# Meryx/ComputeRayTracer

Measured on AMD Instinct MI355X. Metric: Mrays/sec (+ HBM GB/s vs peak), 1080p 250k-tri scene, 1/2/4/8 MI355X, higher is better.
Workload: dtype f32; 1 GPU; S2 atrium250k: 253952 triangles + cornell walls/light, 1920x1080, 64 spp per step (BASELINE config 3)

## Files before the change

### computeraytracer_amd/csrc/crt_api.cpp

```cpp
#include <hip/hip_runtime.h>

#include <algorithm>
#include <cfloat>
#include <cmath>
#include <cstdarg>
#include <cstdio>
#include <cstdlib>
#include <cstring>
#include <chrono>
#include <string>
#include <thread>
#include <vector>

#include "../../include/crt.h"
#include "crt_bvh.h"
#include "crt_device.h"
#include "crt_math.h"

namespace crt {
hipError_t launch_trace(const TraceParams &P, bool count, bool brute, hipStream_t stream);
hipError_t launch_trace_adaptive(const TraceParams &P, const AsTiles &A, bool count, bool brute, hipStream_t stream);
hipError_t wf_launch_resolve_adaptive(const WfParams &P, const AsTiles &A, uint32_t call_end, hipStream_t s);
hipError_t as_launch_select(const AsParams &A, bool compact, hipStream_t s);
hipError_t as_launch_commit(uint32_t *counts, const uint32_t *active, uint32_t n_active, uint32_t samples, hipStream_t s);
// ... 101 lines not shown
    Bvh4 bvh4;
    Bvh4Q bvh4q;
    Bvh8Q bvh8q;
    int quantize = 1;
    int wf_width = 4;

    DevBuf<unsigned char> d_raw;
    DevBuf<float4> d_prim, d_primD, d_nodes, d_nodes4, d_lights;
    DevBuf<int> w_overflow;
    DevBuf<uint4> d_nodes4q, d_nodes8q;
    DevBuf<uint32_t> d_slot_of_index;
    DevBuf<float> d_spectra, d_cie;
    DevScene sc{};

    uint32_t x0 = 0, y0 = 0, tw = 0, th = 0;
    uint32_t band = 0x40000000u, stride = 1, phase = 0;
    DevBuf<float4> d_accum;
    DevBuf<uchar4> d_rgba;
    DevBuf<uchar4> d_frames;
    uint32_t frame_ring = 0;
    std::vector<uint8_t> frame_batch;
    hipStream_t read_stream = nullptr;
    uint32_t ring_from = 1;
    uint32_t resolved_upto = 0;
    float4 *accum_bound = nullptr;
    uchar4 *rgba_bound = nullptr;
    uint32_t sample = 0;
    uint32_t published = 0;
    uint32_t pending = 0;
    bool in_publish = false;
    int wf_cohort = 16;

    DevBuf<unsigned long long> d_counters;
    bool counting = false;
    float last_ms = 0.0f;
    uint32_t last_launches = 0;
    bool last_timed = false;
    uint32_t spp_per_launch = 0;

    int pipeline = 1;
    uint32_t wf_pool = 0;
    uint32_t wf_waves_per_cu = 0;
    int num_cu = 0;
    DevBuf<float4> w_ray_o, w_ray_d, w_sh_d, w_beta, w_radiance, w_nee, w_staging[kWfRing], w_recA, w_recB;
    DevBuf<uint4> w_rng, w_misc, w_recC;
    DevBuf<float2> w_hit;
    DevBuf<uint32_t> w_vis, w_dead, w_tea;
    static constexpr int kMaxPipes = 4;
    int wf_pipes = 2;
    int wf_defer = 1;
    int wf_tail_walk = 1;
    int wf_gen_blocks = 128;
    int wf_trace_form = 2;
    int wf_chunk = 1;
    int wf_ahead = 3;
    int wf_ring = 32;
    int wf_pool_spp = 8;
    double wf_feed = 1.0;
    WfRun *run = nullptr;
    uint32_t wf_finish_at = 32768;
    uint32_t wf_flush_at = 4096;
    uint32_t wf_side_ppw = 64, wf_flush_ppw = 4;
    DevBuf<WfCtl> w_ctl[kMaxPipes];
    DevBuf<WfWorkQ> w_wq;
    static constexpr int kStatusSlots = 64;
    WfStatus *h_status[kMaxPipes] = {};
    WfStatus *d_status[kMaxPipes] = {};
    hipEvent_t ev_status[kMaxPipes][kStatusSlots] = {};
    hipEvent_t ev_done[kMaxPipes][kStatusSlots] = {};
    uint32_t *h_dropped = nullptr;
    bool wf_host_ready = false;
    hipStream_t pipe_stream[kMaxPipes] = {};
    hipStream_t pub_stream = nullptr;
    static constexpr int kFinishStreams = 3;
    hipStream_t fin_stream[kFinishStreams] = {};
    hipEvent_t ev_fin[kFinishStreams] = {};
    int fin_next = 0;
    hipEvent_t ev_fork = nullptr, ev_join[kMaxPipes] = {}, ev_pub_join[kMaxPipes] = {};
    hipEvent_t ev_evict[kMaxPipes][kWfRing] = {};
    hipEvent_t ev_resolved[kWfRing] = {};
    hipEvent_t ev_pub[kWfRing] = {};
    bool time_kernels = false;
    std::vector<hipEvent_t> kev;
    float last_trace_kernel_ms = 0.0f;
    uint32_t last_trace_kernel_launches = 0;
    uint32_t last_iterations = 0;
    unsigned long long probes[8] = {0};

    DevBuf<float4> dn_gbuf;
    DevBuf<uint32_t> dn_key;
    bool dn_valid = false;
    DevBuf<float4> dn_c[2];
    DevBuf<uchar4> dn_rgba;

    float s_prims = 0.0f;
    float tree_pad = 0.0f;
    bool accel_stale = false;
    bool rf_ready = false;
    DevBuf<int> rf_lv2, rf_lv4;
    std::vector<uint32_t> rf_off2, rf_off4;
    DevBuf<uint32_t> rf_nch4, rf_cnt;
    DevBuf<float> rf_fb;

    bool as_on = false;
    bool as_broken = false;
    DevBuf<uint32_t> as_counts;
// ... 1078 lines not shown
        r.K = g.K; r.P = g.P; r.Pp = g.Pp; r.list_cap = g.list_cap;
        r.trace_blocks = (uint32_t)c->num_cu * wf_waves(c);
        r.open.clear();
        WfBatch nb;
        nb.n = n; nb.last_sample = last_sample; nb.id = 0; nb.as_commit = as ? as->commit : 0u;
        r.open.push_back(nb);
        r.seg_total[0] = work_total; r.seg_wps[0] = work_per_shard;
        for (uint32_t b = 0; b < kWfRing; b++) {
            r.queue_left[b] = false; r.consumed[b] = 0; r.resolved_recorded[b] = false;
            for (int p = 0; p < crt_ctx::kMaxPipes; p++) r.listed_until[b][p] = 0;
        }
        r.queue_left[0] = r.work_left = true;
        r.consumed_total = 0; r.rate_consumed = 0; r.rate_its = 0;
        r.per_it = (double)g.Pp;
        r.all_evicting = false; r.poll_next = 0;
        r.as = as ? AsTiles{c->as_active.p, c->as_counts.p, c->as_q.p, as->n_active} : AsTiles{};
        for (int p = 0; p < r.K; p++) {
            const uint32_t it0 = r.pipes[p].it + 2u * (uint32_t)kStatusRing;
            r.pipes[p] = WfPipe();
            r.pipes[p].it = r.pipes[p].it_first = r.pipes[p].it_confirmed = r.pipes[p].it_done = it0;
            r.pipes[p].chunk = (uint32_t)c->wf_chunk;
            WfParams &W = r.pipes[p].W;
            W.sc = c->sc;
            W.ray_o = c->w_ray_o.p; W.ray_d = c->w_ray_d.p; W.sh_d = c->w_sh_d.p; W.beta = c->w_beta.p;
            W.radiance = c->w_radiance.p; W.nee = c->w_nee.p; W.rng = c->w_rng.p; W.misc = c->w_misc.p;
            W.hit = c->w_hit.p; W.vis = c->w_vis.p;
            W.dead = c->w_dead.p + (g.list_per_pipe / 8) * (size_t)p;
            W.rearm = 0;
            W.gen_blocks = std::max(1u, std::min((uint32_t)c->wf_gen_blocks, g.list_cap / 64u));
            W.recA = c->w_recA.p + g.list_per_pipe * (size_t)p; W.recB = c->w_recB.p + g.list_per_pipe * (size_t)p;
            W.recC = c->w_recC.p + g.list_per_pipe * (size_t)p;
            for (uint32_t b = 0; b < kWfRing; b++) {
                W.staging[b] = c->w_staging[b < r.ring ? b : 0].p;
                W.side_base[b] = (b * (uint32_t)crt_ctx::kMaxPipes + (uint32_t)p) * kWfSideCap;
                W.seg[b] = WfSeg{0, 64, 0};
                W.seg_order[b] = 0;
            }
            W.batch_id = 0; W.count_alive = 0; W.keep_pool = 0; W.evict_mask = 0; W.status_out = nullptr;
            W.ctl = c->w_ctl[p].p; W.wq = c->w_wq.p;
            W.slot_base = side_slots + g.Pp * (uint32_t)p; W.reset_wq = (p == 0) ? 1u : 0u;
            W.P = g.Pp; W.x0 = c->x0; W.y0 = c->y0; W.tw = c->tw; W.th = c->th;
            W.band = c->band; W.stride = c->stride; W.phase = c->phase;
            W.tiles_x = g.tiles_x; W.tiles_y = g.tiles_y; W.npix_padded = g.npix_padded;
            W.list_cap = g.list_cap;
            W.seg[0] = WfSeg{work_total, work_per_shard, first_sample};
            W.seg_n = 1;
            W.n_samples = n;
            W.accum = accum_ptr(c); W.rgba = rgba_ptr(c);
            W.tea = c->w_tea.p;
            W.count = c->counting ? 1u : 0u;
            W.overflow_lanes = (uint32_t)c->num_cu * wf_waves(c) * 64u;
            W.stack_overflow = c->w_overflow.p + (size_t)p * W.overflow_lanes * kWfOverflowLevels;
            W.trace_form = (uint32_t)c->wf_trace_form;
            if (!c->pipe_stream[p]) {
                int least = 0, greatest = 0;
                HIPCHK(c, hipDeviceGetStreamPriorityRange(&least, &greatest));
                HIPCHK(c, hipStreamCreateWithPriority(&c->pipe_stream[p], hipStreamNonBlocking, greatest));
            }
            r.pipes[p].stream = c->pipe_stream[p];
            r.pipes[p].blocks_now = r.trace_blocks;
        }
        for (int p = 0; p < r.K; p++) r.rate_its += r.pipes[p].it_confirmed;
        HIPCHK(c, wf_launch_init(r.pipes[0].W, c->stream));
        HIPCHK(c, wf_launch_tea(r.pipes[0].W, c->w_tea.p, c->stream));
        HIPCHK(c, hipEventRecord(c->ev_fork, c->stream));
        for (int p = 0; p < r.K; p++) {
            HIPCHK(c, hipStreamWaitEvent(r.pipes[p].stream, c->ev_fork, 0));
            if (p > 0) HIPCHK(c, wf_launch_init(r.pipes[p].W, r.pipes[p].stream));
        }
        HIPCHK(c, hipStreamWaitEvent(c->pub_stream, c->ev_fork, 0));
        r.live = true;
    } else {
        rc = wf_pump(c, true);
        if (rc) return rc;
        WfBatch nb;
        nb.n = n; nb.last_sample = last_sample; nb.id = (r.open.back().id + 1u) % r.ring; nb.as_commit = as ? as->commit : 0u;
        const uint32_t id = nb.id;
        r.seg_total[id] = work_total; r.seg_wps[id] = work_per_shard;
        r.queue_left[id] = r.work_left = true;
        r.consumed[id] = 0;
        for (int p = 0; p < r.K; p++) {
            WfPipe &pp = r.pipes[p];
            nb.from_it[p] = 0xFFFFFFFFu;
            pp.W.seg[id] = WfSeg{work_total, work_per_shard, first_sample};
            pp.W.n_samples = n;
            pp.W.batch_id = id; pp.W.keep_pool = 1;
            pp.tail_bound = 0; pp.blocks_now = r.trace_blocks;
            pp.any = false; pp.chunk = (uint32_t)c->wf_chunk; pp.done = false;
            pp.dry[id] = false; pp.alive_valid[id] = false; pp.alive[id] = 0;
        }
        for (int p = 0; p < r.K; p++)
            if (r.listed_until[id][p] > r.pipes[p].it_confirmed) {
                HIPCHK(c, hipEventRecord(c->ev_pub_join[p], r.pipes[p].stream));
                HIPCHK(c, hipStreamWaitEvent(c->pub_stream, c->ev_pub_join[p], 0));
            }
        if (r.resolved_recorded[id]) HIPCHK(c, hipStreamWaitEvent(c->pub_stream, c->ev_resolved[id], 0));
        for (int p = 0; p < r.K; p++) HIPCHK(c, wf_launch_init(r.pipes[p].W, c->pub_stream));
        HIPCHK(c, hipEventRecord(c->ev_pub[id], c->pub_stream));
        nb.ready = false;
        r.open.push_back(nb);
    }
    if (!as) c->published += n;
    rc = wf_pump(c, false);
    if (rc == CRT_OK && !defer) rc = wf_flush(c);
    if (rc != CRT_OK && r.live) {
        for (int p = 0; p < crt_ctx::kMaxPipes; p++) if (c->pipe_stream[p]) (void)hipStreamSynchronize(c->pipe_stream[p]);
// ... 679 lines not shown
        c->last_trace_kernel_launches = 0;
    } else {
        HIPCHK(c, hipEventElapsedTime(&total, c->ev0, c->ev1));
        n = c->last_launches;
    }
    if (ms) *ms = total;
    if (launches) *launches = n;
    return CRT_OK;
}

int crt_accel_stats(crt_ctx *c, uint64_t out[8])
{
    if (!c || !out) return CRT_EINVAL;
    const bool wide = c->pipeline == 1 && c->accel_mode == CRT_ACCEL_BVH2 && c->bvh4.n_inner > 0;
    const bool wide8 = wide && c->bvh8q.ok;
    out[4] = wide ? (c->bvh4q.ok ? 16 : 32) : 32;
    out[5] = wide8 ? 8 : wide ? 4 : 2;
    out[6] = wide8 ? c->bvh8q.n_inner : wide ? c->bvh4.n_inner : c->bvh.n_inner;
    out[7] = (uint64_t)c->accel_builder;
    out[0] = c->bvh.n_inner; out[1] = c->bvh.n_leaves; out[2] = c->bvh.max_depth;
    out[3] = (uint64_t)c->bvh.n_inner * 64u + (uint64_t)c->bvh4.n_inner * 128u + (uint64_t)c->prims.size() * 48u;
    return CRT_OK;
}

int crt_set_option(crt_ctx *c, const char *name, int64_t value)
{
    if (!c || !name) return CRT_EINVAL;
    { int rc_ = wf_flush(c); if (rc_) return rc_; }
    if (!std::strcmp(name, "debug_fail_alloc")) { g_fail_alloc_in = value; return CRT_OK; }
    if (!std::strcmp(name, "wf_defer")) { c->wf_defer = value != 0; return CRT_OK; }
    if (!std::strcmp(name, "spp_per_launch")) { c->spp_per_launch = (uint32_t)std::max<int64_t>(0, value); return CRT_OK; }
    if (!std::strcmp(name, "pipeline")) { c->pipeline = value ? 1 : 0; return CRT_OK; }
    if (!std::strcmp(name, "quantize")) { c->quantize = value ? 1 : 0; return CRT_OK; }
    if (!std::strcmp(name, "wf_width")) { c->wf_width = value == 4 ? 4 : 8; return CRT_OK; }
    if (!std::strcmp(name, "wf_finish_at")) { c->wf_finish_at = (uint32_t)std::max<int64_t>(0, value); return CRT_OK; }
    if (!std::strcmp(name, "wf_flush_at")) { c->wf_flush_at = (uint32_t)std::max<int64_t>(0, value); return CRT_OK; }
    if (!std::strcmp(name, "wf_side_ppw")) { c->wf_side_ppw = (uint32_t)std::min<int64_t>(64, std::max<int64_t>(1, value)); return CRT_OK; }
    if (!std::strcmp(name, "wf_flush_ppw")) { c->wf_flush_ppw = (uint32_t)std::min<int64_t>(64, std::max<int64_t>(1, value)); return CRT_OK; }
    if (!std::strcmp(name, "wf_ring")) { c->wf_ring = (int)std::min<int64_t>((int64_t)kWfRing, std::max<int64_t>(2, value)); return CRT_OK; }
    if (!std::strcmp(name, "wf_chunk")) { c->wf_chunk = (int)std::min<int64_t>(16, std::max<int64_t>(1, value)); return CRT_OK; }
    if (!std::strcmp(name, "wf_cohort")) { c->wf_cohort = (int)std::min<int64_t>(256, std::max<int64_t>(1, value)); return CRT_OK; }
    if (!std::strcmp(name, "wf_ahead")) { c->wf_ahead = (int)std::min<int64_t>(32, std::max<int64_t>(2, value)); return CRT_OK; }
    if (!std::strcmp(name, "wf_pool_spp")) { c->wf_pool_spp = (int)std::min<int64_t>(64, std::max<int64_t>(1, value)); return CRT_OK; }
    if (!std::strcmp(name, "wf_feed_pct")) { c->wf_feed = (double)std::min<int64_t>(400, std::max<int64_t>(10, value)) / 100.0; return CRT_OK; }
    if (!std::strcmp(name, "wf_tail_walk")) { c->wf_tail_walk = value != 0; return CRT_OK; }
    if (!std::strcmp(name, "frame_ring")) {
        c->frame_ring = (uint32_t)std::min<int64_t>(256, std::max<int64_t>(0, value));
        c->ring_from = c->sample + 1u;
        if (c->have_scene) { HIPCHK(c, hipSetDevice(c->device)); HIPCHK(c, hipStreamSynchronize(c->stream)); return alloc_frames(c); }
        return CRT_OK;
    }
    if (!std::strcmp(name, "wf_gen_blocks")) { c->wf_gen_blocks = (int)std::min<int64_t>(4096, std::max<int64_t>(1, value)); return CRT_OK; }
    if (!std::strcmp(name, "wf_trace_form")) { c->wf_trace_form = value == 1 ? 1 : 2; return CRT_OK; }
    if (!std::strcmp(name, "wf_pipes")) { c->wf_pipes = (int)std::min<int64_t>(crt_ctx::kMaxPipes, std::max<int64_t>(1, value)); return CRT_OK; }
    if (!std::strcmp(name, "wf_pool")) { c->wf_pool = (uint32_t)std::max<int64_t>(0, value); return CRT_OK; }
    if (!std::strcmp(name, "wf_waves_per_cu")) { c->wf_waves_per_cu = (uint32_t)std::min<int64_t>(32, std::max<int64_t>(0, value)); return CRT_OK; }
    if (!std::strcmp(name, "time_kernels")) {
        c->time_kernels = value != 0; c->last_trace_kernel_launches = 0;
        HIPCHK(c, hipSetDevice(c->device));
        while (value > 1 && c->kev.size() < 2 * (size_t)std::min<int64_t>(value, 1 << 20)) {
            hipEvent_t e;
            HIPCHK(c, hipEventCreate(&e));
            c->kev.push_back(e);
        }
        return CRT_OK;
    }
    return fail(c, CRT_EINVAL, "crt_set_option: unknown option '%s'", name);
}

static int dn_check_state(crt_ctx *c, const char *what)
{
    if (!c->have_scene || c->accel_mode < 0) return fail(c, CRT_ESTATE, "%s: scene + accel required", what);
    if (c->accel_stale) return fail(c, CRT_ESTATE, "%s: primitives were updated: call crt_refit_accel or crt_build_accel first", what);
    if (c->sample == 0) return fail(c, CRT_ESTATE, "%s: no sample traced yet", what);
    if (c->band != 0x40000000u)
        return fail(c, CRT_ESTATE, "%s: not under a row-band partition (neighbouring local rows are not neighbouring image rows)", what);
    if ((size_t)c->tw * c->th != 0 && !accum_ptr(c))
        return fail(c, CRT_ENOMEM, "%s: the tile's buffers are not allocated (an earlier crt_set_tile failed)", what);
    return CRT_OK;
}

static int dn_ensure_gbuffer(crt_ctx *c)
{
    if (c->dn_valid) return CRT_OK;
    const size_t n = (size_t)c->tw * c->th;
    if (c->dn_gbuf.n < 2 * n) HIPCHK(c, c->dn_gbuf.alloc(2 * n));
    if (c->dn_key.n < n) HIPCHK(c, c->dn_key.alloc(n));
    HIPCHK(c, dn_launch_gbuffer(c->sc, c->x0, c->y0, c->tw, c->th, c->dn_gbuf.p, c->dn_key.p, c->accel_mode == CRT_ACCEL_NONE, c->stream));
    c->dn_valid = true;
    return CRT_OK;
}

int crt_denoise(crt_ctx *c, const crt_denoise_params *params, float *rgb_out, uint8_t *rgba8_out)
{
    if (!c) return CRT_EINVAL;
    const crt_denoise_params dp = params ? *params : crt_denoise_params{5u, 1.0f, 0.5f, 0.3f};
    if (dp.iterations > 10u) return fail(c, CRT_EINVAL, "crt_denoise: iterations %u > 10", dp.iterations);
    const float sig[3] = {dp.sigma_color, dp.sigma_normal, dp.sigma_plane};
    for (float v : sig)
        if (!(v > 0.0f && v <= 3.40282347e38f)) return fail(c, CRT_EINVAL, "crt_denoise: every sigma must be positive and finite");
    if (c->as_on) return as_refuse(c, "crt_denoise");
    { int rc = dn_check_state(c, "crt_denoise"); if (rc) return rc; }
    HIPCHK(c, hipSetDevice(c->device));
    { int rc_ = wf_flush(c); if (rc_) return rc_; }
    const size_t n = (size_t)c->tw * c->th;
    if (n) {
// ... 253 lines not shown
```

### computeraytracer_amd/csrc/crt_device.h

```cpp
#pragma once
#include <hip/hip_runtime.h>
#include <stdint.h>

namespace crt {

constexpr uint32_t kNoHit = 0xFFFFFFFFu;
constexpr int kStackDepth = 64;
constexpr uint32_t kNLambda = 301;
constexpr uint32_t kNCie = 471;
constexpr int CRT_NCOUNTERS_DEV = 16;

struct DevScene {
    const float4 *prim;
    const float4 *primD;
    const uint32_t *slot_of_index;
    const float4 *nodes;
    const float4 *nodes4;
    const uint4 *nodes4q;
    const uint4 *nodes8q;
    const float *spectra;
    const float *cie;
    const float4 *lights;
    uint32_t nprim;
    uint32_t npatch;
// ... 85 lines not shown
    unsigned long long rays;
    unsigned long long consumed[kWfRing];
    uint32_t left[kWfRing];
    uint32_t alive[kWfRing];
};

constexpr uint32_t kWfFinishSegs = 32;
struct WfFinishSegs {
    struct WfCtl *ctl[kWfFinishSegs];
    uint32_t base[kWfFinishSegs], batch[kWfFinishSegs];
    uint32_t n, blocks_per_seg;
};

struct WfParams {
    DevScene sc;
    float4 *ray_o, *ray_d, *sh_d, *beta, *radiance, *nee;
    uint4 *rng, *misc;
    float2 *hit;
    uint32_t *vis;
    float4 *recA, *recB;
    uint4 *recC;
    uint32_t *dead;
    uint32_t rearm;
    uint32_t gen_blocks;
    float4 *staging[kWfRing];
    uint32_t batch_id;
    WfStatus *status_out;
    uint32_t count_alive;
    uint32_t keep_pool;
    uint32_t side_base[kWfRing];
    uint32_t evict_mask;
    WfCtl *ctl;
    WfWorkQ *wq;
    WfSeg seg[kWfRing];
    uint32_t seg_order[kWfRing];
    uint32_t seg_n;
    uint32_t slot_base;
    uint32_t reset_wq;
    uint32_t P;
    uint32_t x0, y0, tw, th;
    uint32_t band, stride, phase;
    uint32_t tiles_x, tiles_y;
    uint32_t npix_padded;
    uint32_t list_cap;
    uint32_t tail_bound;
    uint32_t n_samples;
    float4 *accum;
    uchar4 *rgba;
    uchar4 *frames;
    uint32_t frame_ring;
    const uint32_t *tea;
    uint32_t count;
    uint32_t trace_form;
    int *stack_overflow;
    uint32_t overflow_lanes;
};

}
```

### computeraytracer_amd/csrc/crt_wavefront.hip

```cpp
#include "crt_shade.h"
#include <algorithm>

namespace crt {

#ifndef CRT_WF_STACK
#define CRT_WF_STACK 32
#endif
#ifndef CRT_WF_REFILL
#define CRT_WF_REFILL 24
#endif
#ifndef CRT_WF_INNER_RUN
#define CRT_WF_INNER_RUN 6
#endif
#ifndef CRT_WF_BURSTS
#define CRT_WF_BURSTS 4
#endif
#ifndef CRT_WF_BVH4
#define CRT_WF_BVH4 1
#endif
#ifndef CRT_WF_LEAF_AT
#define CRT_WF_LEAF_AT 32
#endif
#ifndef CRT_WF_SPEC
#define CRT_WF_SPEC 1
// ... 1051 lines not shown
#endif
                }
            }
        }
    }
    if (COUNT) {
        wave_add(ctl->counters[blockIdx.x % kWfShards] + CRT_CNT_NODES, c_nodes);
        wave_add(ctl->counters[blockIdx.x % kWfShards] + CRT_CNT_PRIMS, c_prims);
        if (lane == 0) {
            atomicAdd(ctl->counters[blockIdx.x % kWfShards] + 8, (unsigned long long)d_inner_it); atomicAdd(ctl->counters[blockIdx.x % kWfShards] + 9, (unsigned long long)d_inner_act);
            atomicAdd(ctl->counters[blockIdx.x % kWfShards] + 10, (unsigned long long)d_leaf_it); atomicAdd(ctl->counters[blockIdx.x % kWfShards] + 11, (unsigned long long)d_leaf_act);
            atomicAdd(ctl->counters[blockIdx.x % kWfShards] + 12, (unsigned long long)d_prim_it); atomicAdd(ctl->counters[blockIdx.x % kWfShards] + 13, (unsigned long long)d_scans); atomicAdd(ctl->counters[blockIdx.x % kWfShards] + 14, (unsigned long long)d_refill);
            atomicAdd(ctl->counters[blockIdx.x % kWfShards] + 15, (unsigned long long)d_refill_lanes);
        }
    }
}

#ifndef CRT_WF_PICK_AT
#define CRT_WF_PICK_AT 8
#endif
#ifndef CRT_WF_PKFMA
#define CRT_WF_PKFMA 0
#endif
#ifndef CRT_WF_LEAF2_AT
#define CRT_WF_LEAF2_AT 28
#endif
#ifndef CRT_WF_STALL_AT
#define CRT_WF_STALL_AT 16
#endif
constexpr int kStk2 = 16;
#ifndef CRT_WF_RING
#define CRT_WF_RING 32
#endif
constexpr uint32_t kRing2 = CRT_WF_RING;

__device__ __forceinline__ int stack_pop2(const int *stk, const int *ovf, size_t ovl, int sp)
{
    int v = stk[(sp < kStk2 ? sp : kStk2 - 1) * 64];
    if (sp >= kStk2) v = *(const volatile int *)(ovf + (size_t)(sp - kStk2) * ovl);
    return v;
}
__device__ __forceinline__ uint32_t mbcnt64(unsigned long long m)
{
    return __builtin_amdgcn_mbcnt_hi((uint32_t)(m >> 32), __builtin_amdgcn_mbcnt_lo((uint32_t)m, 0u));
}
__device__ __forceinline__ unsigned long long hit_key(float t, uint32_t index)
{
    return ((unsigned long long)f_bits(t) << 32) | (unsigned long long)(index == kNoHit ? 0xFFFFFFFFu : 0xFFFFFFFEu - index);
}

#ifndef CRT_WF_T2_WAVES
#define CRT_WF_T2_WAVES 5
#endif
template <bool COUNT>
__global__ __launch_bounds__(64, CRT_WF_T2_WAVES) void k_wf_trace2(const WfParams P, uint32_t it)
{
    __shared__ int lds_stack[kStk2 * 64];
    __shared__ float4 ring[4][kRing2];
    __shared__ uint2 ring_l[kRing2];
    __shared__ unsigned long long cell[64];
    __shared__ uint32_t cslot[64];
    __shared__ uint2 tasks[64];
    WfCtl *ctl = P.ctl;
    const uint4 *__restrict__ nodesq = P.sc.nodes4q;
    const f3 qscale = f3{P.sc.qscale[0], P.sc.qscale[1], P.sc.qscale[2]}, qbase = f3{P.sc.qbase[0], P.sc.qbase[1], P.sc.qbase[2]};
    const float4 *__restrict__ prim = P.sc.prim;
    const float4 *__restrict__ primD = P.sc.primD;
    uint32_t *__restrict__ g_vis = P.vis;
    float2 *__restrict__ g_hit = P.hit;
    const size_t cls_stride = (size_t)P.list_cap * kWfShards;
    const float4 *__restrict__ recA = P.recA + (size_t)((it & 1u) * 4u) * cls_stride;
    const float4 *__restrict__ recB = P.recB + (size_t)((it & 1u) * 4u) * cls_stride;
    const uint4 *__restrict__ recC = P.recC + (size_t)((it & 1u) * 4u) * cls_stride;
    const float hit_pad = P.sc.hit_pad;
    const int root = P.sc.root4;
    int *__restrict__ ovf = P.stack_overflow + ((size_t)blockIdx.x * 64 + lane_id());
    const size_t ovl = P.overflow_lanes;
    const uint32_t nprim = P.sc.nprim;
    const bool fetchD = ((unsigned long long)P.sc.npatch << CRT_WF_PATCH_RECOMPUTE) > (unsigned long long)nprim;
    DevScene S = P.sc;
    S.prim = prim; S.primD = primD;

    const uint32_t ringi = it & 3u;
    const uint32_t lane = lane_id();
    int *stk = lds_stack + lane;
    const float t_min = 0.001f;

    uint32_t cur_shard = blockIdx.x % kWfShards, sh_e0 = 0, sh_e1 = 0, sh_e2 = 0, sh_total = 0;
    uint32_t chunk_pos = 0, chunk_end = 0, ring_head = 0, ring_n = 0;
    bool have_shard = false, exhausted = false;
    {
        const WfShard &so = ctl->shard[ringi][cur_shard];
        sh_e0 = so.n[0]; sh_e1 = sh_e0 + so.n[1]; sh_e2 = sh_e1 + so.n[2]; sh_total = sh_e2 + so.n[3];
        have_shard = sh_total > 0u;
    }
    bool active = false;
    int pend = 0;
    f3 o = f3{0, 0, 0}, d = f3{0, 0, 0}, id = f3{0, 0, 0}, oid = f3{0, 0, 0};
    uint32_t excl = 0, slot = 0, b_index = kNoHit, b_slot = kNoHit, b_slot_in = kNoHit;
    float t_max = 0.0f;
    bool shadow = false;
    int node = kNoNode, sp = 0;
    bool gx = false, gy = false, gz = false;
    uint32_t c_nodes = 0, c_prims = 0;
    uint32_t d_inner_it = 0, d_inner_act = 0, d_leaf_it = 0, d_leaf_act = 0, d_prim_it = 0, d_refill = 0, d_refill_lanes = 0, d_scans = 0;

    for (;;) {
        const unsigned long long idle = __ballot(!active);
        const int nidle = __popcll(idle);
        if (nidle >= CRT_WF_PICK_AT) {
            if (ring_n == 0u && !exhausted) {
                for (int guard = 0; chunk_pos == chunk_end && !exhausted && guard < 2 * (int)kWfShards; guard++) {
                    if (have_shard) {
                        uint32_t base = 0;
                        if (lane == 0) base = atomicAdd(&ctl->shard[ringi][cur_shard].cur, (uint32_t)kTraceChunk);
                        base = __shfl(base, 0, 64);
                        if (base < sh_total) { chunk_pos = base; chunk_end = min(base + (uint32_t)kTraceChunk, sh_total); break; }
                        have_shard = false;
                    }
                    if (COUNT) d_scans++;
                    const WfShard &sl = ctl->shard[ringi][lane % kWfShards];
                    const uint32_t e0 = sl.n[0], e1 = e0 + sl.n[1], e2 = e1 + sl.n[2], tot = e2 + sl.n[3];
                    const uint32_t cur_l = __hip_atomic_load(&sl.cur, __ATOMIC_RELAXED, __HIP_MEMORY_SCOPE_AGENT);
                    const unsigned long long avail = __ballot(cur_l < tot);
                    if (!avail) { exhausted = true; break; }
                    const uint32_t rot = cur_shard & 63u;
                    const unsigned long long rmask = rot ? ((avail >> rot) | (avail << (64u - rot))) : avail;
                    cur_shard = ((uint32_t)(__ffsll((long long)rmask) - 1) + rot) & 63u;
                    sh_e0 = __shfl(e0, (int)cur_shard, 64); sh_e1 = __shfl(e1, (int)cur_shard, 64);
                    sh_e2 = __shfl(e2, (int)cur_shard, 64); sh_total = __shfl(tot, (int)cur_shard, 64);
                    have_shard = true;
                }
                if (chunk_pos < chunk_end) {
                    const uint32_t n = min(kRing2, chunk_end - chunk_pos);
                    bool ok = false;
                    float4 R0 = float4{0, 0, 0, 0}, R1 = R0, R2 = R0, R3 = R0;
                    uint2 RL = uint2{kNoHit, kNoHit};
                    if (lane < n) {
                        const uint32_t idx = chunk_pos + lane;
                        const size_t region = (size_t)cur_shard * P.list_cap;
                        const bool sh = idx >= sh_e1;
                        const size_t g = idx < sh_e0 ? region + idx : idx < sh_e1 ? cls_stride + region + (idx - sh_e0)
                                       : idx < sh_e2 ? 2u * cls_stride + region + (idx - sh_e1) : 3u * cls_stride + region + (idx - sh_e2);
                        const float4 ro = ldnt(&recA[g]), rd = ldnt(&recB[g]);
                        uint4 rc = uint4{0, 0, 0, 0};
                        if (sh) rc = ldnt(&recC[g]);
                        uint32_t r_slot;
                        float r_tmax;
                        ok = true;
                        if (sh) {
                            r_slot = rc.x & kWfListSlot; r_tmax = rd.w;
                            RL = uint2{rc.y, rc.z};
                        } else {
                            r_slot = f_bits(rd.w) & kWfListSlot; r_tmax = CRT_INFINITY;
                            if (f_bits(rd.w) & kWfListAlsoExt) ok = false;
                            else if (nprim == 0u) { g_hit[r_slot] = float2{r_tmax, bits_f(kNoHit)}; ok = false; }
                        }
// ... 88 lines not shown
                    else if (sp > 0) { sp--; node = stack_pop2(stk, ovf, ovl, sp); }
                    else node = kNoNode;
                }
                const f3 to = f3{__shfl(o.x, owner, 64), __shfl(o.y, owner, 64), __shfl(o.z, owner, 64)};
                const f3 td = f3{__shfl(d.x, owner, 64), __shfl(d.y, owner, 64), __shfl(d.z, owner, 64)};
                const uint32_t t_excl = (uint32_t)__shfl((int)excl, owner, 64);
                bool acc = false;
                unsigned long long key = 0;
                if (lane < T) {
                    const unsigned long long cur = cell[owner];
                    float tm = bits_f((uint32_t)(cur >> 32));
                    const uint32_t low = (uint32_t)cur;
                    uint32_t bi = low == 0xFFFFFFFFu ? kNoHit : 0xFFFFFFFEu - low;
                    const uint32_t bs0 = low == 0xFFFFFFFFu ? kNoHit : 0xFFFFFFFEu;
                    uint32_t bs = bs0;
                    if ((f_bits(A.w) & 3u) == 2u) tri_test(A, B, C, ps, to, td, t_excl, t_min, hit_pad, tm, bi, bs);
                    else {
                        if (!fetchD && (f_bits(A.w) & 3u) == 0u) { const f3 nn = normalize(cross(xyz(B), xyz(C))); D = float4{nn.x, nn.y, nn.z, dot(xyz(B), xyz(B))}; }
                        hit_test_rec<false>(A, B, C, D, hit_pad, ps, to, td, t_excl, t_min, tm, bi, bs);
                    }
                    if (COUNT && __ballot((f_bits(A.w) & 3u) != 2u) != 0ull) d_scans += 64u;
                    acc = bs != bs0;
                    if (acc) {
                        key = hit_key(tm, bi);
                        atomicMin(&cell[owner], key);
                    }
                    if (COUNT) c_prims++;
                }
                __builtin_amdgcn_fence(__ATOMIC_ACQ_REL, "wavefront");
                __builtin_amdgcn_wave_barrier();
                if (acc && cell[owner] == key) cslot[owner] = ps;
                __builtin_amdgcn_fence(__ATOMIC_ACQ_REL, "wavefront");
                __builtin_amdgcn_wave_barrier();
                if (incl) {
                    const unsigned long long v = cell[lane];
                    const uint32_t low = (uint32_t)v;
                    t_max = bits_f((uint32_t)(v >> 32));
                    b_index = low == 0xFFFFFFFFu ? kNoHit : 0xFFFFFFFEu - low;
                    b_slot = cslot[lane];
                    bool done = false;
                    if (shadow && b_slot != b_slot_in) done = true;
                    else if (node == kNoNode && pend == 0) done = true;
                    if (done) {
                        if (shadow) stnt(&g_vis[slot], (b_slot == b_slot_in) ? 1u : 0u);
                        else stnt(&g_hit[slot], float2{t_max, bits_f(b_slot)});
                        active = false;
                    }
                }
            } else {
                if (COUNT) { d_inner_it++; d_inner_act += (uint32_t)ni; }
                if (inner) {
                    float k0, k1, k2, k3;
                    int r0, r1, r2, r3;
                    const uint4 *nq = (const uint4 *)((const char *)nodesq + ((uint32_t)node << 6));
                    const uint4 Q0 = nq[0], Q1 = nq[1], Q2 = nq[2], Q3 = nq[3];
                    const uint32_t nxa = gx ? Q1.z : Q0.x, nxb = gx ? Q1.w : Q0.y, fxa = gx ? Q0.x : Q1.z, fxb = gx ? Q0.y : Q1.w;
                    const uint32_t nya = gy ? Q2.x : Q0.z, nyb = gy ? Q2.y : Q0.w, fya = gy ? Q0.z : Q2.x, fyb = gy ? Q0.w : Q2.y;
                    const uint32_t nza = gz ? Q2.z : Q1.x, nzb = gz ? Q2.w : Q1.y, fza = gz ? Q1.x : Q2.z, fzb = gz ? Q1.y : Q2.w;
#if CRT_WF_PKFMA
                    {
                        const v2f ix = v2f{id.x, id.x}, iy = v2f{id.y, id.y}, iz = v2f{id.z, id.z};
                        const v2f ox = v2f{oid.x, oid.x}, oy = v2f{oid.y, oid.y}, oz = v2f{oid.z, oid.z};
#define CRT_PK(Q, I, O) __builtin_elementwise_fma(v2f{(float)((Q) & 0xFFFFu), (float)((Q) >> 16)}, I, O)
                        const v2f tnx_a = CRT_PK(nxa, ix, ox), tnx_b = CRT_PK(nxb, ix, ox), tfx_a = CRT_PK(fxa, ix, ox), tfx_b = CRT_PK(fxb, ix, ox);
                        const v2f tny_a = CRT_PK(nya, iy, oy), tny_b = CRT_PK(nyb, iy, oy), tfy_a = CRT_PK(fya, iy, oy), tfy_b = CRT_PK(fyb, iy, oy);
                        const v2f tnz_a = CRT_PK(nza, iz, oz), tnz_b = CRT_PK(nzb, iz, oz), tfz_a = CRT_PK(fza, iz, oz), tfz_b = CRT_PK(fzb, iz, oz);
#undef CRT_PK
#define CRT_QK(K, NX, NY, NZ, FX, FY, FZ) { \
                            const float tn_ = __builtin_fmaxf(__builtin_fmaxf(NX, NY), __builtin_fmaxf(NZ, t_min)); \
                            const float tf_ = __builtin_fminf(__builtin_fminf(FX, FY), __builtin_fminf(FZ, t_max)); \
                            K = (tn_ <= tf_ * 1.0000005f) ? tn_ : 3.0e38f; }
                        CRT_QK(k0, tnx_a.x, tny_a.x, tnz_a.x, tfx_a.x, tfy_a.x, tfz_a.x)
                        CRT_QK(k1, tnx_a.y, tny_a.y, tnz_a.y, tfx_a.y, tfy_a.y, tfz_a.y)
                        CRT_QK(k2, tnx_b.x, tny_b.x, tnz_b.x, tfx_b.x, tfy_b.x, tfz_b.x)
                        CRT_QK(k3, tnx_b.y, tny_b.y, tnz_b.y, tfx_b.y, tfy_b.y, tfz_b.y)
#undef CRT_QK
                    }
#else
#define CRT_QBOX(K, NXQ, NYQ, NZQ, FXQ, FYQ, FZQ) { \
                        const float tn_ = __builtin_fmaxf(__builtin_fmaxf(fma_((float)(NXQ), id.x, oid.x), fma_((float)(NYQ), id.y, oid.y)), \
                                                          __builtin_fmaxf(fma_((float)(NZQ), id.z, oid.z), t_min)); \
                        const float tf_ = __builtin_fminf(__builtin_fminf(fma_((float)(FXQ), id.x, oid.x), fma_((float)(FYQ), id.y, oid.y)), \
                                                          __builtin_fminf(fma_((float)(FZQ), id.z, oid.z), t_max)); \
                        K = (tn_ <= tf_ * 1.0000005f) ? tn_ : 3.0e38f; }
                    CRT_QBOX(k0, nxa & 0xFFFFu, nya & 0xFFFFu, nza & 0xFFFFu, fxa & 0xFFFFu, fya & 0xFFFFu, fza & 0xFFFFu)
                    CRT_QBOX(k1, nxa >> 16, nya >> 16, nza >> 16, fxa >> 16, fya >> 16, fza >> 16)
                    CRT_QBOX(k2, nxb & 0xFFFFu, nyb & 0xFFFFu, nzb & 0xFFFFu, fxb & 0xFFFFu, fyb & 0xFFFFu, fzb & 0xFFFFu)
                    CRT_QBOX(k3, nxb >> 16, nyb >> 16, nzb >> 16, fxb >> 16, fyb >> 16, fzb >> 16)
#undef CRT_QBOX
#endif
                    r0 = (int)Q3.x; r1 = (int)Q3.y; r2 = (int)Q3.z; r3 = (int)Q3.w;
                    if (COUNT) c_nodes += 4;
#define CRT_CAS(ka, ra, kb, rb) { const bool sw_ = kb < ka; const float tk_ = sw_ ? kb : ka; kb = sw_ ? ka : kb; ka = tk_; \
                                  const int tr_ = sw_ ? rb : ra; rb = sw_ ? ra : rb; ra = tr_; }
                    CRT_CAS(k0, r0, k1, r1) CRT_CAS(k2, r2, k3, r3) CRT_CAS(k0, r0, k2, r2) CRT_CAS(k1, r1, k3, r3) CRT_CAS(k1, r1, k2, r2)
#undef CRT_CAS
                    if (k0 < 3.0e38f) {
                        if (k3 < 3.0e38f) { if (sp < kStk2) stk[sp * 64] = r3; else ovf[(size_t)(sp - kStk2) * ovl] = r3; sp++; }
                        if (k2 < 3.0e38f) { if (sp < kStk2) stk[sp * 64] = r2; else ovf[(size_t)(sp - kStk2) * ovl] = r2; sp++; }
                        if (k1 < 3.0e38f) { if (sp < kStk2) stk[sp * 64] = r1; else ovf[(size_t)(sp - kStk2) * ovl] = r1; sp++; }
                        node = r0;
                    } else if (sp > 0) {
                        sp--; node = stack_pop2(stk, ovf, ovl, sp);
                    } else {
                        node = kNoNode;
                        if (pend == 0) {
                            if (shadow) stnt(&g_vis[slot], (b_slot == b_slot_in) ? 1u : 0u);
                            else stnt(&g_hit[slot], float2{t_max, bits_f(b_slot)});
                            active = false;
                        }
                    }
                }
            }
        }
    }
    if (COUNT) {
        wave_add(ctl->counters[blockIdx.x % kWfShards] + CRT_CNT_NODES, c_nodes);
        wave_add(ctl->counters[blockIdx.x % kWfShards] + CRT_CNT_PRIMS, c_prims);
        if (lane == 0) {
            atomicAdd(ctl->counters[blockIdx.x % kWfShards] + 8, (unsigned long long)d_inner_it); atomicAdd(ctl->counters[blockIdx.x % kWfShards] + 9, (unsigned long long)d_inner_act);
            atomicAdd(ctl->counters[blockIdx.x % kWfShards] + 10, (unsigned long long)d_leaf_it); atomicAdd(ctl->counters[blockIdx.x % kWfShards] + 11, (unsigned long long)d_leaf_act);
            atomicAdd(ctl->counters[blockIdx.x % kWfShards] + 12, (unsigned long long)d_prim_it); atomicAdd(ctl->counters[blockIdx.x % kWfShards] + 13, (unsigned long long)d_scans); atomicAdd(ctl->counters[blockIdx.x % kWfShards] + 14, (unsigned long long)d_refill);
            atomicAdd(ctl->counters[blockIdx.x % kWfShards] + 15, (unsigned long long)d_refill_lanes);
        }
    }
}

template <bool COUNT>
__global__ __launch_bounds__(64) void k_wf_finish(const WfParams P, const WfFinishSegs G)
{
    __shared__ int lds_stack[kStackDepth * 64];
    const DevScene &S = P.sc;
    const uint32_t seg = blockIdx.x / G.blocks_per_seg, blk = blockIdx.x % G.blocks_per_seg;
    WfCtl *ctl = G.ctl[seg];
    int *stk = lds_stack + lane_id();
    const uint32_t j = blk * P.tail_bound + threadIdx.x;
    const uint32_t count = min(ctl->side_count[G.batch[seg]], kWfSideCap);
    if (blk == 0 && threadIdx.x == 0 && count > G.blocks_per_seg * P.tail_bound) atomicAdd(&ctl->dropped, count - G.blocks_per_seg * P.tail_bound);
    const bool mine = threadIdx.x < P.tail_bound && j < count;
    const uint32_t slot = G.base[seg] + (mine ? j : 0u);
    uint32_t flags = 0;
    if (mine) flags = P.misc[slot].y;
    bool alive = mine && (flags & kWfAlive);
    bool pend_sh = false, pend_ext = false;
    const bool wide = S.nodes4q != nullptr && S.nodes8q == nullptr;
    ShadeCnt cn;
    uint32_t c_nodes = 0, c_prims = 0;
    for (int guard = 0; guard < 512 && __ballot(alive) != 0ull; guard++) {
        if (alive) {
            const float4 ro = P.ray_o[slot];
            const f3 o = xyz(ro);
            const uint32_t excl = f_bits(ro.w);
            if (pend_sh) {
                const float4 sd = P.sh_d[slot];
                float t_max = sd.w;
                uint32_t b_index = P.vis[slot];
                const uint32_t l_slot = S.slot_of_index[b_index];
                uint32_t b_slot = l_slot;
                if (!wide || !traverse4q<COUNT>(S, stk, o, xyz(sd), excl, true, t_max, b_index, b_slot, c_nodes, c_prims))
                    traverse<COUNT>(S, stk, o, xyz(sd), excl, true, t_max, b_index, b_slot, c_nodes, c_prims);
                P.vis[slot] = (b_slot == l_slot) ? 1u : 0u;
            }
            if (pend_ext) {
                const float4 rd = P.ray_d[slot];
                if (f_bits(rd.w) == 0u) {
                    float t_max = CRT_INFINITY;
                    uint32_t b_index = kNoHit, b_slot = kNoHit;
                    if (!wide || !traverse4q<COUNT>(S, stk, o, xyz(rd), excl, false, t_max, b_index, b_slot, c_nodes, c_prims))
                        traverse<COUNT>(S, stk, o, xyz(rd), excl, false, t_max, b_index, b_slot, c_nodes, c_prims);
                    P.hit[slot] = float2{t_max, bits_f(b_slot)};
                }
            }
            ShadeOut so = shade_body<COUNT, true>(P, slot, true, cn);
            const uint32_t resolved = shade_store<COUNT, true>(P, slot, true, so, cn);
            (void)resolved;
            alive = so.alive; pend_ext = so.emit_ext; pend_sh = so.emit_sh;
        }
// ... 74 lines not shown
                for (int k = 0; k < 4; k++) c->shard[r][i].n[k] = 0;
                c->shard[r][i].cur = 0; c->shard[r][i].n_dead = 0;
                for (uint32_t b = 0; b < kWfRing; b++) c->shard[r][i].alive[b] = 0;
            }
        if (i == 0) { if (P.keep_pool) c->side_count[P.batch_id] = 0; else for (uint32_t b = 0; b < kWfRing; b++) c->side_count[b] = 0; }
        if (P.reset_wq) {
            P.wq[P.batch_id].work[i].cur = 0;
            if (i == 0) {
                P.wq[P.batch_id].work_done = 0;
                P.wq[P.batch_id].work_per_shard = P.seg[P.batch_id].work_per_shard;
                P.wq[P.batch_id].work_total = P.seg[P.batch_id].work_total;
            }
        }
    }
}

hipError_t wf_launch_init(const WfParams &P, hipStream_t s)
{
    hipLaunchKernelGGL(k_wf_init, dim3(P.keep_pool ? 1u : (P.P + 255) / 256), dim3(256), 0, s, P);
    return hipGetLastError();
}

hipError_t wf_launch_tea(const WfParams &P, uint32_t *out, hipStream_t s)
{
    const size_t npix = (size_t)P.tw * P.th;
    if (npix == 0) return hipSuccess;
    hipLaunchKernelGGL(k_wf_tea, dim3((unsigned)((npix + 255) / 256)), dim3(256), 0, s, P, out);
    return hipGetLastError();
}

hipError_t wf_launch_shade(const WfParams &P, uint32_t it, hipStream_t s)
{
    const uint32_t bps = (4u * P.tail_bound + CRT_WF_SHADE_BLOCK - 1u) / CRT_WF_SHADE_BLOCK;
    const dim3 gs(P.tail_bound ? kWfShards * bps : (P.P + CRT_WF_SHADE_BLOCK - 1) / CRT_WF_SHADE_BLOCK), bs(CRT_WF_SHADE_BLOCK);
    if (P.count) hipLaunchKernelGGL((k_wf_shade<true>), gs, bs, 0, s, P, it);
    else hipLaunchKernelGGL((k_wf_shade<false>), gs, bs, 0, s, P, it);
    return hipGetLastError();
}

hipError_t wf_launch_gen(const WfParams &P, uint32_t it, hipStream_t s, const AsTiles *A)
{
    if (P.gen_blocks == 0u) return hipErrorInvalidValue;
    const dim3 gs(kWfShards * P.gen_blocks), bs(64);
    if (A) {
        if (P.count) hipLaunchKernelGGL((k_wf_gen<true, true>), gs, bs, 0, s, P, it, *A);
        else hipLaunchKernelGGL((k_wf_gen<false, true>), gs, bs, 0, s, P, it, *A);
        return hipGetLastError();
    }
    if (P.count) hipLaunchKernelGGL((k_wf_gen<true, false>), gs, bs, 0, s, P, it, AsTiles{});
    else hipLaunchKernelGGL((k_wf_gen<false, false>), gs, bs, 0, s, P, it, AsTiles{});
    return hipGetLastError();
}

hipError_t wf_launch_trace(const WfParams &P, uint32_t it, uint32_t trace_blocks, hipStream_t s)
{
    const dim3 g(trace_blocks), b(64);
    const int q = !CRT_WF_BVH4 ? 0 : P.sc.nodes8q != nullptr ? 2 : P.sc.nodes4q != nullptr ? 1 : 0;
    if (q == 1 && P.trace_form == 2u) {
        if (P.count) hipLaunchKernelGGL((k_wf_trace2<true>), g, b, 0, s, P, it);
        else hipLaunchKernelGGL((k_wf_trace2<false>), g, b, 0, s, P, it);
        return hipGetLastError();
    }
    if (P.count) {
        if (q == 2) hipLaunchKernelGGL((k_wf_trace<true, 2>), g, b, 0, s, P, it);
        else if (q == 1) hipLaunchKernelGGL((k_wf_trace<true, 1>), g, b, 0, s, P, it);
        else hipLaunchKernelGGL((k_wf_trace<true, 0>), g, b, 0, s, P, it);
    } else {
        if (q == 2) hipLaunchKernelGGL((k_wf_trace<false, 2>), g, b, 0, s, P, it);
        else if (q == 1) hipLaunchKernelGGL((k_wf_trace<false, 1>), g, b, 0, s, P, it);
        else hipLaunchKernelGGL((k_wf_trace<false, 0>), g, b, 0, s, P, it);
    }
    return hipGetLastError();
}

hipError_t wf_launch_finish(const WfParams &P, WfFinishSegs G, uint32_t max_paths, hipStream_t s)
{
    if (P.tail_bound == 0u || P.tail_bound > 64u || G.n > kWfFinishSegs) return hipErrorInvalidValue;
    G.blocks_per_seg = (std::min(max_paths, kWfSideCap) + P.tail_bound - 1u) / P.tail_bound;
    if (G.blocks_per_seg == 0 || G.n == 0) return hipSuccess;
    if (P.count) hipLaunchKernelGGL((k_wf_finish<true>), dim3(G.n * G.blocks_per_seg), dim3(64), 0, s, P, G);
    else hipLaunchKernelGGL((k_wf_finish<false>), dim3(G.n * G.blocks_per_seg), dim3(64), 0, s, P, G);
    return hipGetLastError();
}



hipError_t wf_launch_resolve(const WfParams &P, uint32_t last_sample, hipStream_t s)
{
    const size_t npix = (size_t)P.tw * P.th;
    if (npix == 0) return hipSuccess;
    hipLaunchKernelGGL(k_wf_resolve, dim3((unsigned)((npix + 63) / 64)), dim3(64), 0, s, P, last_sample);
    return hipGetLastError();
}

hipError_t wf_launch_resolve_adaptive(const WfParams &P, const AsTiles &A, uint32_t call_end, hipStream_t s)
{
    if (A.n_active == 0 || !A.active) return hipErrorInvalidValue;
    hipLaunchKernelGGL(k_wf_resolve_as, dim3(A.n_active), dim3(64), 0, s, P, call_end, A);
    return hipGetLastError();
}

}
```

Baseline: 7258 Mrays/s.

## Cache top BVH4 nodes in LDS and pack four waves per trace block

At launch, the trace2 kernel copies the first 21 or 85 BVH4 nodes into dynamic shared memory in a component-transposed layout. Inner-node fetches for those indices then read LDS instead of global memory. The default of 85 also groups four independent persistent waves into one 256-thread block so the cached top levels are shared across waves, with per-wave LDS state and global wave ids. In exchange, each block pays a cooperative preload and barrier, uses more LDS per block (which can reduce occupancy), and adds a branch on every node fetch.

```diff
diff --git a/computeraytracer_amd/csrc/crt_api.cpp b/computeraytracer_amd/csrc/crt_api.cpp
--- a/computeraytracer_amd/csrc/crt_api.cpp
+++ b/computeraytracer_amd/csrc/crt_api.cpp
@@ -177,6 +177,7 @@
     int wf_tail_walk = 1;
     int wf_gen_blocks = 128;
     int wf_trace_form = 2;
+    uint32_t wf_top_nodes = 85;
     int wf_chunk = 1;
     int wf_ahead = 3;
     int wf_ring = 32;
@@ -1361,6 +1362,7 @@
             W.overflow_lanes = (uint32_t)c->num_cu * wf_waves(c) * 64u;
             W.stack_overflow = c->w_overflow.p + (size_t)p * W.overflow_lanes * kWfOverflowLevels;
             W.trace_form = (uint32_t)c->wf_trace_form;
+            W.top_nodes = c->wf_top_nodes;
             if (!c->pipe_stream[p]) {
                 int least = 0, greatest = 0;
                 HIPCHK(c, hipDeviceGetStreamPriorityRange(&least, &greatest));
@@ -2146,6 +2148,10 @@
     }
     if (!std::strcmp(name, "wf_gen_blocks")) { c->wf_gen_blocks = (int)std::min<int64_t>(4096, std::max<int64_t>(1, value)); return CRT_OK; }
     if (!std::strcmp(name, "wf_trace_form")) { c->wf_trace_form = value == 1 ? 1 : 2; return CRT_OK; }
+    if (!std::strcmp(name, "wf_top_nodes")) {
+        if (value != 0 && value != 21 && value != 85) return fail(c, CRT_EINVAL, "crt_set_option: wf_top_nodes is 0, 21 or 85");
+        c->wf_top_nodes = (uint32_t)value; return CRT_OK;
+    }
     if (!std::strcmp(name, "wf_pipes")) { c->wf_pipes = (int)std::min<int64_t>(crt_ctx::kMaxPipes, std::max<int64_t>(1, value)); return CRT_OK; }
     if (!std::strcmp(name, "wf_pool")) { c->wf_pool = (uint32_t)std::max<int64_t>(0, value); return CRT_OK; }
     if (!std::strcmp(name, "wf_waves_per_cu")) { c->wf_waves_per_cu = (uint32_t)std::min<int64_t>(32, std::max<int64_t>(0, value)); return CRT_OK; }
diff --git a/computeraytracer_amd/csrc/crt_device.h b/computeraytracer_amd/csrc/crt_device.h
--- a/computeraytracer_amd/csrc/crt_device.h
+++ b/computeraytracer_amd/csrc/crt_device.h
@@ -161,6 +161,7 @@
     const uint32_t *tea;
     uint32_t count;
     uint32_t trace_form;
+    uint32_t top_nodes;
     int *stack_overflow;
     uint32_t overflow_lanes;
 };
diff --git a/computeraytracer_amd/csrc/crt_wavefront.hip b/computeraytracer_amd/csrc/crt_wavefront.hip
--- a/computeraytracer_amd/csrc/crt_wavefront.hip
+++ b/computeraytracer_amd/csrc/crt_wavefront.hip
@@ -1127,15 +1127,33 @@
 #ifndef CRT_WF_T2_WAVES
 #define CRT_WF_T2_WAVES 5
 #endif
-template <bool COUNT>
-__global__ __launch_bounds__(64, CRT_WF_T2_WAVES) void k_wf_trace2(const WfParams P, uint32_t it)
-{
-    __shared__ int lds_stack[kStk2 * 64];
-    __shared__ float4 ring[4][kRing2];
-    __shared__ uint2 ring_l[kRing2];
-    __shared__ unsigned long long cell[64];
-    __shared__ uint32_t cslot[64];
-    __shared__ uint2 tasks[64];
+struct Trace2Lds {
+    int stack[kStk2 * 64];
+    float4 ring[4][kRing2];
+    uint2 ring_l[kRing2];
+    unsigned long long cell[64];
+    uint32_t cslot[64];
+    uint2 tasks[64];
+};
+extern __shared__ uint4 trace2_top[];
+template <bool COUNT, int TOPK, int NW>
+__global__ __launch_bounds__(64 * NW, CRT_WF_T2_WAVES) void k_wf_trace2(const WfParams P, uint32_t it, uint32_t n_waves)
+{
+    __shared__ Trace2Lds lds[NW];
+    const uint32_t wv = NW > 1 ? (uint32_t)__builtin_amdgcn_readfirstlane((int)(threadIdx.x >> 6)) : 0u;
+    const uint32_t gw = blockIdx.x * (uint32_t)NW + wv;
+    if constexpr (TOPK > 0) {
+        const uint32_t n_top = min((uint32_t)TOPK, P.sc.n_nodes4) * 4u;
+        for (uint32_t i = threadIdx.x; i < n_top; i += 64u * NW) trace2_top[(i & 3u) * TOPK + (i >> 2)] = P.sc.nodes4q[i];
+        __syncthreads();
+    }
+    if (NW > 1 && gw >= n_waves) return;
+    int *lds_stack = lds[wv].stack;
+    float4 (&ring)[4][kRing2] = lds[wv].ring;
+    uint2 (&ring_l)[kRing2] = lds[wv].ring_l;
+    unsigned long long (&cell)[64] = lds[wv].cell;
+    uint32_t (&cslot)[64] = lds[wv].cslot;
+    uint2 (&tasks)[64] = lds[wv].tasks;
     WfCtl *ctl = P.ctl;
     const uint4 *__restrict__ nodesq = P.sc.nodes4q;
     const f3 qscale = f3{P.sc.qscale[0], P.sc.qscale[1], P.sc.qscale[2]}, qbase = f3{P.sc.qbase[0], P.sc.qbase[1], P.sc.qbase[2]};
@@ -1149,7 +1167,7 @@
     const uint4 *__restrict__ recC = P.recC + (size_t)((it & 1u) * 4u) * cls_stride;
     const float hit_pad = P.sc.hit_pad;
     const int root = P.sc.root4;
-    int *__restrict__ ovf = P.stack_overflow + ((size_t)blockIdx.x * 64 + lane_id());
+    int *__restrict__ ovf = P.stack_overflow + ((size_t)gw * 64 + lane_id());
     const size_t ovl = P.overflow_lanes;
     const uint32_t nprim = P.sc.nprim;
     const bool fetchD = ((unsigned long long)P.sc.npatch << CRT_WF_PATCH_RECOMPUTE) > (unsigned long long)nprim;
@@ -1161,7 +1179,7 @@
     int *stk = lds_stack + lane;
     const float t_min = 0.001f;
 
-    uint32_t cur_shard = blockIdx.x % kWfShards, sh_e0 = 0, sh_e1 = 0, sh_e2 = 0, sh_total = 0;
+    uint32_t cur_shard = gw % kWfShards, sh_e0 = 0, sh_e1 = 0, sh_e2 = 0, sh_total = 0;
     uint32_t chunk_pos = 0, chunk_end = 0, ring_head = 0, ring_n = 0;
     bool have_shard = false, exhausted = false;
     {
@@ -1178,6 +1196,9 @@
     int node = kNoNode, sp = 0;
     bool gx = false, gy = false, gz = false;
     uint32_t c_nodes = 0, c_prims = 0;
+#ifdef CRT_WF_PROBE
+    uint32_t h_top[3] = {0, 0, 0};
+#endif
     uint32_t d_inner_it = 0, d_inner_act = 0, d_leaf_it = 0, d_leaf_act = 0, d_prim_it = 0, d_refill = 0, d_refill_lanes = 0, d_scans = 0;
 
     for (;;) {
@@ -1372,8 +1393,13 @@
                 if (inner) {
                     float k0, k1, k2, k3;
                     int r0, r1, r2, r3;
-                    const uint4 *nq = (const uint4 *)((const char *)nodesq + ((uint32_t)node << 6));
-                    const uint4 Q0 = nq[0], Q1 = nq[1], Q2 = nq[2], Q3 = nq[3];
+                    uint4 Q0, Q1, Q2, Q3;
+                    if (TOPK > 0 && node < TOPK) {
+                        Q0 = trace2_top[node]; Q1 = trace2_top[TOPK + node]; Q2 = trace2_top[2 * TOPK + node]; Q3 = trace2_top[3 * TOPK + node];
+                    } else {
+                        const uint4 *nq = (const uint4 *)((const char *)nodesq + ((uint32_t)node << 6));
+                        Q0 = nq[0]; Q1 = nq[1]; Q2 = nq[2]; Q3 = nq[3];
+                    }
                     const uint32_t nxa = gx ? Q1.z : Q0.x, nxb = gx ? Q1.w : Q0.y, fxa = gx ? Q0.x : Q1.z, fxb = gx ? Q0.y : Q1.w;
                     const uint32_t nya = gy ? Q2.x : Q0.z, nyb = gy ? Q2.y : Q0.w, fya = gy ? Q0.z : Q2.x, fyb = gy ? Q0.w : Q2.y;
                     const uint32_t nza = gz ? Q2.z : Q1.x, nzb = gz ? Q2.w : Q1.y, fza = gz ? Q1.x : Q2.z, fzb = gz ? Q1.y : Q2.w;
@@ -1411,6 +1437,9 @@
 #endif
                     r0 = (int)Q3.x; r1 = (int)Q3.y; r2 = (int)Q3.z; r3 = (int)Q3.w;
                     if (COUNT) c_nodes += 4;
+#ifdef CRT_WF_PROBE
+                    if (COUNT) { h_top[0] += node < 21; h_top[1] += node < 85; h_top[2] += node < 341; }
+#endif
 #define CRT_CAS(ka, ra, kb, rb) { const bool sw_ = kb < ka; const float tk_ = sw_ ? kb : ka; kb = sw_ ? ka : kb; ka = tk_; \
                                   const int tr_ = sw_ ? rb : ra; rb = sw_ ? ra : rb; ra = tr_; }
                     CRT_CAS(k0, r0, k1, r1) CRT_CAS(k2, r2, k3, r3) CRT_CAS(k0, r0, k2, r2) CRT_CAS(k1, r1, k3, r3) CRT_CAS(k1, r1, k2, r2)
@@ -1435,14 +1464,20 @@
         }
     }
     if (COUNT) {
-        wave_add(ctl->counters[blockIdx.x % kWfShards] + CRT_CNT_NODES, c_nodes);
-        wave_add(ctl->counters[blockIdx.x % kWfShards] + CRT_CNT_PRIMS, c_prims);
+        wave_add(ctl->counters[gw % kWfShards] + CRT_CNT_NODES, c_nodes);
+        wave_add(ctl->counters[gw % kWfShards] + CRT_CNT_PRIMS, c_prims);
         if (lane == 0) {
-            atomicAdd(ctl->counters[blockIdx.x % kWfShards] + 8, (unsigned long long)d_inner_it); atomicAdd(ctl->counters[blockIdx.x % kWfShards] + 9, (unsigned long long)d_inner_act);
-            atomicAdd(ctl->counters[blockIdx.x % kWfShards] + 10, (unsigned long long)d_leaf_it); atomicAdd(ctl->counters[blockIdx.x % kWfShards] + 11, (unsigned long long)d_leaf_act);
-            atomicAdd(ctl->counters[blockIdx.x % kWfShards] + 12, (unsigned long long)d_prim_it); atomicAdd(ctl->counters[blockIdx.x % kWfShards] + 13, (unsigned long long)d_scans); atomicAdd(ctl->counters[blockIdx.x % kWfShards] + 14, (unsigned long long)d_refill);
-            atomicAdd(ctl->counters[blockIdx.x % kWfShards] + 15, (unsigned long long)d_refill_lanes);
-        }
+            atomicAdd(ctl->counters[gw % kWfShards] + 8, (unsigned long long)d_inner_it); atomicAdd(ctl->counters[gw % kWfShards] + 9, (unsigned long long)d_inner_act);
+            atomicAdd(ctl->counters[gw % kWfShards] + 10, (unsigned long long)d_leaf_it); atomicAdd(ctl->counters[gw % kWfShards] + 11, (unsigned long long)d_leaf_act);
+            atomicAdd(ctl->counters[gw % kWfShards] + 12, (unsigned long long)d_prim_it);
+#ifndef CRT_WF_PROBE
+            atomicAdd(ctl->counters[gw % kWfShards] + 13, (unsigned long long)d_scans); atomicAdd(ctl->counters[gw % kWfShards] + 14, (unsigned long long)d_refill);
+            atomicAdd(ctl->counters[gw % kWfShards] + 15, (unsigned long long)d_refill_lanes);
+#endif
+        }
+#ifdef CRT_WF_PROBE
+        for (int k = 0; k < 3; k++) wave_add(ctl->counters[gw % kWfShards] + 13 + k, h_top[k]);
+#endif
     }
 }
 
@@ -1623,14 +1658,26 @@
     return hipGetLastError();
 }
 
+template <int TOPK, int NW>
+static hipError_t launch_trace2(const WfParams &P, uint32_t it, uint32_t n_waves, hipStream_t s)
+{
+    const dim3 g((n_waves + NW - 1u) / NW), b(64 * NW);
+    if (P.count) hipLaunchKernelGGL((k_wf_trace2<true, TOPK, NW>), g, b, 64 * TOPK, s, P, it, n_waves);
+    else hipLaunchKernelGGL((k_wf_trace2<false, TOPK, NW>), g, b, 64 * TOPK, s, P, it, n_waves);
+    return hipGetLastError();
+}
+
 hipError_t wf_launch_trace(const WfParams &P, uint32_t it, uint32_t trace_blocks, hipStream_t s)
 {
     const dim3 g(trace_blocks), b(64);
     const int q = !CRT_WF_BVH4 ? 0 : P.sc.nodes8q != nullptr ? 2 : P.sc.nodes4q != nullptr ? 1 : 0;
     if (q == 1 && P.trace_form == 2u) {
-        if (P.count) hipLaunchKernelGGL((k_wf_trace2<true>), g, b, 0, s, P, it);
-        else hipLaunchKernelGGL((k_wf_trace2<false>), g, b, 0, s, P, it);
-        return hipGetLastError();
+        switch (P.top_nodes) {
+        case 0u: return launch_trace2<0, 1>(P, it, trace_blocks, s);
+        case 21u: return launch_trace2<21, 1>(P, it, trace_blocks, s);
+        case 85u: return launch_trace2<85, 4>(P, it, trace_blocks, s);
+        default: return hipErrorInvalidValue;
+        }
     }
     if (P.count) {
         if (q == 2) hipLaunchKernelGGL((k_wf_trace<true, 2>), g, b, 0, s, P, it);
```

After: 5993 Mrays/s, median of 2. 0.826x the previous value.
